# ruanjue/bsalign

Hardware: AMD Instinct MI355X
Metric: GCUPS (giga band-cell updates / s), 8-bit banded striped global alignment (higher is better)
Workload: dtype i8

## Files before the change

### bsalign_amd/__init__.py

```python
import ctypes as C
import os
import sys

import numpy as np

_HERE = os.path.dirname(os.path.abspath(__file__))
LIB_PATH = os.environ.get("BSA_LIB_PATH") or os.path.join(_HERE, "libbsalign_hip.so")

MODE_GLOBAL, MODE_OVERLAP, MODE_EXTEND = 0, 1, 2
MODE_ROWRECORDS, MODE_SCORE_ONLY, MODE_SEQ2BIT = 0x100, 0x400, 0x800
MODE_CIGAR_EQX = 0x1000
MODE_QSTRAND = 0x2000
MODE_BAND_MARGIN = 0x4000
ST_MARGIN_SHIFT, ST_MARGIN_NONE = 16, 0xFFFF
QOFF_REVCOMP = 1 << 63
CIGAR_M, CIGAR_I, CIGAR_D, CIGAR_EQ, CIGAR_X = 0, 1, 2, 7, 8
ST_BAD_BASE, ST_EMPTY, ST_TRACE, ST_DEVICE = 1, 2, 4, 8
KMER_CHAIN_DEVICE = 1
KMER_STRAND_AUTO = 2
ST_REVCOMP = 16
WINDOW_NONE = 0xFFFFFFFF

E_NAMES = {0: "OK", -1: "BSA_E_NODEVICE", -2: "BSA_E_ARG", -3: "BSA_E_NOMEM", -4: "BSA_E_HIP",
           -5: "BSA_E_CIGAR_CAP", -6: "BSA_E_UNSUPPORTED"}
# ... 51 lines not shown
class KmerParams(C.Structure):
    _fields_ = [("ksz", C.c_uint32), ("threads", C.c_uint32)]


RESULT_DTYPE = np.dtype([(n, np.int32) for n in ("score", "qb", "qe", "tb", "te", "mat", "mis", "ins", "del", "aln")])

_lib = None


DIAGDP_PROB_DTYPE = np.dtype([("seq0", np.uint64), ("seq1", np.uint64), ("mats0", np.uint64, (4,)), ("mats1", np.uint64, (4,)),
                              ("out0", np.uint64), ("out1", np.uint64), ("mlen", np.uint32), ("mbeg", np.uint32), ("mend", np.uint32), ("W", np.uint32)])


def build():
    import subprocess
    subprocess.run(["make", "-s", "-C", os.path.join(_HERE, "csrc"), "all"], check=True)


def lib():
    global _lib
    if _lib is None:
        if not os.path.exists(LIB_PATH):
            raise RuntimeError("libbsalign_hip.so is not built (run `python -c 'import __graft_entry__ as g; g.build()'`); "
                               "there is no CPU fallback")
        if "torch" not in sys.modules and not os.environ.get("BSA_NO_TORCH_PRELOAD"):
            try:
                import torch
            except ImportError:
                pass
        L = C.CDLL(LIB_PATH)
        vp, u8p, u32p, u64p = C.c_void_p, C.c_void_p, C.c_void_p, C.c_void_p
        L.bsa_ctx_create.argtypes = [C.c_int, C.POINTER(vp)]
        L.bsa_ctx_destroy.argtypes = [vp]
        L.bsa_ctx_destroy.restype = None
        L.bsa_ctx_set_stream.argtypes = [vp, vp]
        L.bsa_ctx_set_workspace_limit.argtypes = [vp, C.c_size_t]
        L.bsa_ctx_sync.argtypes = [vp]
        L.bsa_last_error.argtypes = [vp]
        L.bsa_last_error.restype = C.c_char_p
        L.bsa_ctx_last_kernel_ms.argtypes = [vp, C.POINTER(C.c_double), C.POINTER(C.c_long), C.POINTER(C.c_double)]
        L.bsa_ctx_last_trace_ms.argtypes = [vp, C.POINTER(C.c_double), C.POINTER(C.c_long)]
        L.bsa_ctx_last_margin_ms.argtypes = [vp, C.POINTER(C.c_double), C.POINTER(C.c_long)]
        L.bsa_ctx_last_kernel_name.argtypes = [vp, C.c_int]
        L.bsa_ctx_last_kernel_name.restype = C.c_char_p
        L.bsa_ctx_last_handover.argtypes = [vp]
        L.bsa_ctx_last_handover.restype = C.c_long
        L.bsa_set_score_matrix.argtypes = [C.POINTER(C.c_int8), C.c_int8, C.c_int8]
        L.bsa_set_score_matrix.restype = None
        L.bsa_align_batch.argtypes = [vp, u8p, C.c_size_t, u64p, u32p, u64p, u32p, C.c_size_t, C.POINTER(AlignParams),
                                      vp, u32p, C.c_size_t, u64p, u32p]
        L.bsa_align_plan_create.argtypes = [vp, u64p, u32p, u64p, u32p, C.c_size_t, C.POINTER(AlignParams), C.POINTER(vp)]
        if hasattr(L, "bsa_align8_abs_form_internal"):
            L.bsa_align8_abs_form_internal.argtypes = [C.POINTER(AlignParams), C.POINTER(C.c_uint32)]
        if hasattr(L, "bsa_align8_flag_span_internal"):
            L.bsa_align8_flag_span_internal.argtypes = [C.POINTER(AlignParams), C.POINTER(C.c_uint32)]
        if hasattr(L, "bsa_align8_x_choice_internal"):
            L.bsa_align8_x_choice_internal.argtypes = [C.POINTER(AlignParams), C.c_uint32, C.c_uint32, C.c_int, C.c_uint32, C.c_int, C.c_uint64, C.c_int,
                                                       C.POINTER(C.c_uint64), C.c_char_p, C.c_size_t]
        L.bsa_align_plan_destroy.argtypes = [vp]
        L.bsa_align_plan_destroy.restype = None
        L.bsa_align_plan_cells.argtypes = [vp]
        L.bsa_align_plan_cells.restype = C.c_double
        L.bsa_align_run.argtypes = [vp, u8p, vp, u32p, C.c_size_t, u64p, u32p]
        L.bsa_synth_stride.argtypes = [C.c_uint32]
        L.bsa_synth_stride.restype = C.c_size_t
        L.bsa_synth_pairs_host.argtypes = [C.c_uint64, C.c_uint64, C.c_size_t, C.c_uint32, C.c_uint32, u8p, u32p]
        L.bsa_synth_pairs_dev.argtypes = [vp, C.c_uint64, C.c_uint64, C.c_size_t, C.c_uint32, C.c_uint32, u8p, u32p]
        L.bsa_seq_pack2bit.argtypes = [vp, u8p, C.c_uint64, u64p, u32p]
        if hasattr(L, "bsa_edit_batch"):
            L.bsa_edit_batch.argtypes = [vp, u8p, C.c_size_t, u64p, u32p, u64p, u32p, C.c_size_t, C.POINTER(EditParams),
                                         vp, u32p, C.c_size_t, u64p, u32p]
            L.bsa_edit_plan_create.argtypes = [vp, u64p, u32p, u64p, u32p, C.c_size_t, C.POINTER(EditParams), C.POINTER(vp)]
            L.bsa_edit_plan_destroy.argtypes = [vp]
            L.bsa_edit_plan_destroy.restype = None
            L.bsa_edit_plan_cells.argtypes = [vp]
            L.bsa_edit_plan_cells.restype = C.c_double
            L.bsa_edit_run.argtypes = [vp, u8p, vp, u32p, C.c_size_t, u64p, u32p]
        if hasattr(L, "bsa_edit_choice_internal"):
            L.bsa_edit_choice_internal.argtypes = [C.c_uint32, C.c_uint32, C.c_uint32, C.c_int, C.c_uint32, C.c_int, C.c_int, C.c_int, C.c_int, C.c_int,
                                                   C.POINTER(C.c_uint64), C.c_char_p, C.c_char_p, C.c_size_t]
        L.bsa_kmer_edit_batch.argtypes = [vp, u8p, C.c_size_t, u64p, u32p, u64p, u32p, C.c_size_t, C.POINTER(KmerParams),
                                          vp, u32p, C.c_size_t, u64p, u32p]
        L.bsa_kmer_edit_batch2.argtypes = [vp, u8p, C.c_size_t, u64p, u32p, u64p, u32p, C.c_size_t, C.POINTER(KmerParams),
                                           vp, u32p, C.c_size_t, u64p, u32p, C.c_uint32]
        L.bsa_kmer_chain_batch.argtypes = [vp, u8p, C.c_size_t, u64p, u32p, u64p, u32p, C.c_size_t, C.c_uint32,
                                           u64p, C.c_size_t, u64p, u32p]
        L.bsa_kmer_chain_batch2.argtypes = [vp, u8p, C.c_size_t, u64p, u32p, u64p, u32p, C.c_size_t, C.c_uint32,
                                            u64p, C.c_size_t, u64p, u32p, C.c_uint32]
        L.bsa_ctx_last_kmer_chain_ms.argtypes = [vp, C.POINTER(C.c_double), C.POINTER(C.c_long), C.POINTER(C.c_long)]
        L.bsa_kmer_chain_plan_create.argtypes = [vp, u64p, u32p, u64p, u32p, C.c_size_t, C.c_uint32, C.c_uint32, C.POINTER(vp)]
        L.bsa_kmer_chain_plan_destroy.argtypes = [vp]
        L.bsa_kmer_chain_plan_destroy.restype = None
        L.bsa_kmer_chain_plan_chunks.argtypes = [vp]
        L.bsa_kmer_chain_plan_chunks.restype = C.c_uint32
        L.bsa_kmer_chain_words_bound.argtypes = [u32p, u32p, C.c_size_t]
        L.bsa_kmer_chain_words_bound.restype = C.c_uint64
        L.bsa_kmer_chain_run.argtypes = [vp, u8p, u64p, C.c_size_t, u64p, u32p]
        L.bsa_cigar_windows_bound.argtypes = [u32p, C.c_size_t, C.c_uint32]
        L.bsa_cigar_windows_bound.restype = C.c_uint64
        L.bsa_cigar_windows_run.argtypes = [vp, vp, u32p, u64p, C.c_size_t, C.c_uint32, vp, C.c_size_t, u64p]
        L.bsa_cigar_windows_batch.argtypes = [vp, vp, u32p, u64p, C.c_size_t, C.c_uint32, vp, C.c_size_t, u64p]
        L.bsa_rows_block_bytes.argtypes = [C.c_uint32, C.c_int8, C.c_int8, C.c_int8, C.c_int8]
        L.bsa_rows_block_bytes.restype = C.c_size_t
        L.bsa_rows_run.argtypes = [vp, vp, vp, C.c_size_t, vp, vp, vp, C.POINTER(RowsParams)]
        L.bsa_sweep_run.argtypes = [vp, vp, vp, vp, C.c_size_t, vp, vp, vp, C.POINTER(SweepParams), vp]
        L.bsa_sweep_host.argtypes = [vp, vp, C.c_size_t, vp, C.c_size_t, vp, vp, vp, C.c_size_t, C.POINTER(SweepParams), vp, C.c_size_t, vp]
        L.bsa_poa_graph_supported.argtypes = [C.POINTER(SweepParams), C.c_uint32]
        L.bsa_poa_graph_host.argtypes = [vp, vp, C.c_size_t, vp, C.c_size_t, vp, C.c_size_t, vp, C.c_size_t, vp, C.c_size_t, C.POINTER(SweepParams),
                                         vp, vp, C.c_size_t, vp, vp]
        L.bsa_poa_graph_run.argtypes = [vp, vp, C.c_size_t, vp, vp, vp, C.c_size_t, vp, C.c_uint32, C.POINTER(SweepParams), vp, vp, vp, vp, vp, vp]
        L.bsa_align_debug_rows.argtypes = [vp, C.c_uint32, u8p, C.c_size_t, C.POINTER(C.c_uint32)]
        L.bsa_diagdp_batch.argtypes = [vp, u8p, C.c_size_t, vp, C.c_size_t, u8p, C.c_size_t]
        L.bsa_diagdp_last_ms.argtypes = [vp]
        L.bsa_diagdp_last_ms.restype = C.c_double
        L.bsa_env_reload.restype = None
        _lib = L
    _sync_env()
    return _lib


_env_seen = None


def _sync_env():
    global _env_seen
    cur = tuple(sorted((k, v) for k, v in os.environ.items() if k.startswith("BSA_")))
    if cur != _env_seen:
        _lib.bsa_env_reload()
        _env_seen = cur


def _np(a, dt):
    return np.ascontiguousarray(a, dtype=dt)


def _p(a):
    return a.ctypes.data_as(C.c_void_p)


def make_params(mode=MODE_GLOBAL, bandwidth=128, M=2, X=-6, O=-3, E=-2, Q=0, P=0, matrix=None):
    p = AlignParams()
    p.mode, p.bandwidth = mode, bandwidth
    if matrix is None:
        lib().bsa_set_score_matrix(p.matrix, M, X)
    else:
        for i in range(16):
            p.matrix[i] = int(matrix[i])
    p.gapo1, p.gape1, p.gapo2, p.gape2 = O, E, Q, P
    return p


def align8_abs_form(par):
    rows = C.c_uint32(0)
    form = lib().bsa_align8_abs_form_internal(C.byref(par), C.byref(rows))
    return int(form), int(rows.value)


FLAG_SPAN_TERMS = ("M: f - d", "D: d - E", "D: f - E", "D: d - E, row -1", "D: f - E, row -1", "R, Od")


def align8_flag_span(par):
    terms = (C.c_uint32 * len(FLAG_SPAN_TERMS))()
    span = lib().bsa_align8_flag_span_internal(C.byref(par), terms)
    return int(span), tuple(int(v) for v in terms)


X_CHOICE_FIELDS = ("form", "W", "L", "pw", "do2", "score", "abs", "m3", "wps", "rebase_rows", "grid", "groups", "nseg", "seg_rows", "spin_cap", "rmask", "ctl_bytes",
                   "state_bytes", "n8", "nb8", "gap_model", "xq_need")
X_NONE, X_STATIC, X_SEG, X_WHOLE, X_MIX = range(5)


def align8_x_choice(par, count, max_tlen, static_band=False, code_fmt=0, score=False, xq_bytes=0, cus=256):
    out = (C.c_uint64 * len(X_CHOICE_FIELDS))()
    name = C.create_string_buffer(400)
    rc = lib().bsa_align8_x_choice_internal(C.byref(par), count, max_tlen, int(static_band), code_fmt, int(score), xq_bytes, cus, out, name, len(name))
    if rc < 0:
        raise ValueError("bsa_align8_x_choice_internal: bad arguments")
    d = dict(zip(X_CHOICE_FIELDS, (int(v) for v in out)))
    d.update(name=name.value.decode(), launch=rc == 1)
    return d


EDIT_CHOICE_FIELDS = tuple("fwd%d_%s" % (i, f) for i in (0, 1) for f in ("form", "n", "tiled", "track", "lanes", "grid", "block")) \
    + ("trace_form", "trace_tiled", "trace_lanes", "trace_grid", "row_fmt")
E_NONE, E_REG, E_GRP, E_GRP32, E_WIDE, E_GEN = range(6)
T_NONE, T_WAVE, T_PLAIN, T_COOP = range(4)


def edit_choice(bw, wide, count, mode=MODE_GLOBAL, bandwidth=0, score=False, alone=True, cus=256, occ_plain=8, occ_coop=8):
    out = (C.c_uint64 * len(EDIT_CHOICE_FIELDS))()
    fwd, trace = C.create_string_buffer(200), C.create_string_buffer(200)
    rc = lib().bsa_edit_choice_internal(bw, wide, count, mode, bandwidth, int(score), int(alone), cus, occ_plain, occ_coop, out, fwd, trace, 200)
    if rc < 0:
        raise ValueError("bsa_edit_choice_internal: bad arguments")
    d = dict(zip(EDIT_CHOICE_FIELDS, (int(v) for v in out)))
    d.update(fwd_name=fwd.value.decode(), trace_name=trace.value.decode(), launch=rc == 1)
    return d


def pack2bit(codes):
    c = np.ascontiguousarray(codes, dtype=np.uint8).ravel()
    nw = (c.size + 31) // 32
    buf = np.zeros(nw * 32, dtype=np.uint64)
    buf[:c.size] = c & 3
    shift = np.uint64(62) - np.uint64(2) * np.arange(32, dtype=np.uint64)
    return np.bitwise_or.reduce(buf.reshape(nw, 32) << shift, axis=1).astype(np.uint64)


def unpack2bit(words, off, n):
    i = np.uint64(off) + np.arange(n, dtype=np.uint64)
# ... 465 lines not shown
```

### bsalign_amd/csrc/bsa_align8_x.hip

```cpp
#include "bsa_common.h"
#include "bsa_dpp.h"
#include <algorithm>
#include <cstdio>
typedef short xv2s __attribute__((ext_vector_type(2)));
typedef unsigned short xv2u __attribute__((ext_vector_type(2)));
static __device__ __forceinline__ uint32_t x_add(uint32_t a, uint32_t b){ return __builtin_bit_cast(uint32_t, (xv2u)(__builtin_bit_cast(xv2u, a) + __builtin_bit_cast(xv2u, b))); }
static __device__ __forceinline__ uint32_t x_sub(uint32_t a, uint32_t b){ return __builtin_bit_cast(uint32_t, (xv2u)(__builtin_bit_cast(xv2u, a) - __builtin_bit_cast(xv2u, b))); }
static __device__ __forceinline__ uint32_t x_max(uint32_t a, uint32_t b){ return __builtin_bit_cast(uint32_t, __builtin_elementwise_max(__builtin_bit_cast(xv2s, a), __builtin_bit_cast(xv2s, b))); }
typedef _Float16 xv2h __attribute__((ext_vector_type(2)));
static __device__ __forceinline__ uint32_t x_max3(uint32_t a, uint32_t b, uint32_t c){
	return __builtin_bit_cast(uint32_t, __builtin_elementwise_maximum(__builtin_elementwise_maximum(__builtin_bit_cast(xv2h, a), __builtin_bit_cast(xv2h, b)), __builtin_bit_cast(xv2h, c)));
}
static __device__ __forceinline__ uint32_t x_minu(uint32_t a, uint32_t b){ return __builtin_bit_cast(uint32_t, __builtin_elementwise_min(__builtin_bit_cast(xv2u, a), __builtin_bit_cast(xv2u, b))); }
static __device__ __forceinline__ uint32_t x_satsubu(uint32_t a, uint32_t b){ return __builtin_bit_cast(uint32_t, __builtin_elementwise_sub_sat(__builtin_bit_cast(xv2u, a), __builtin_bit_cast(xv2u, b))); }
static __device__ __forceinline__ uint32_t x_acc(uint32_t acc, uint32_t flag, uint32_t two){
	return __builtin_bit_cast(uint32_t, (xv2u)(__builtin_bit_cast(xv2u, acc) * __builtin_bit_cast(xv2u, two) + __builtin_bit_cast(xv2u, flag)));
}
static __device__ __forceinline__ uint32_t x_ins(uint32_t acc, uint32_t n, uint32_t bit){ return __builtin_amdgcn_bitop3_b32(n, acc, bit, 0x4E); }
static __device__ __forceinline__ uint32_t x_ins0(uint32_t n, uint32_t bit){ return __builtin_amdgcn_bitop3_b32(n, n, bit, 0x0A); }
static __device__ __forceinline__ uint32_t x_shl15(uint32_t a){ return __builtin_bit_cast(uint32_t, (xv2u)(__builtin_bit_cast(xv2u, a) << 15)); }
static __device__ __forceinline__ uint32_t x_ashr8(uint32_t a){ return __builtin_bit_cast(uint32_t, (xv2s)(__builtin_bit_cast(xv2s, a) >> 8)); }
static __device__ __forceinline__ uint32_t x_shl8(uint32_t a){ return __builtin_bit_cast(uint32_t, (xv2u)(__builtin_bit_cast(xv2u, a) << 8)); }
static __device__ __forceinline__ void x_sel(uint32_t &x, uint32_t y, uint64_t take){ asm("v_cndmask_b32 %0, %0, %1, %2" : "+v"(x) : "v"(y), "s"(take)); }
static __device__ __forceinline__ uint32_t x_q8(int v){ return (((uint32_t)v & 0xffu) << 8) * 0x00010001u; }
static __device__ __forceinline__ uint32_t x_i16(int v){ return ((uint32_t)v & 0xffffu) * 0x00010001u; }
static __device__ __forceinline__ int x_lo8(uint32_t x){ return __builtin_amdgcn_sbfe((int)x, 8, 8); }
static __device__ __forceinline__ int x_hi8(uint32_t x){ return (int)x >> 24; }
static __device__ __forceinline__ int x_lo16(uint32_t x){ return __builtin_amdgcn_sbfe((int)x, 0, 16); }
static __device__ __forceinline__ int x_hi16(uint32_t x){ return (int)x >> 16; }

#define XDPP(old, x, ctrl, bank) ((uint32_t)__builtin_amdgcn_update_dpp((int)(old), (int)(x), (ctrl), 0xf, (bank), false))
#define XDPPZ(x, ctrl, bank) ((uint32_t)__builtin_amdgcn_update_dpp(0, (int)(x), (ctrl), 0xf, (bank), true))
#define XQP(a, b, c, d) ((a) | ((b) << 2) | ((c) << 4) | ((d) << 6))
#define XROW_SHL(n) (0x100 + (n))
#define XROW_SHR(n) (0x110 + (n))
#define XHALF_MIRROR 0x141

template<int L> static __device__ __forceinline__ uint32_t x_bcast_first(uint32_t x){
	const uint32_t s = XDPPZ(x, XQP(0, 0, 0, 0), 0xf);
	if constexpr (L == 4) return s;
	else return XDPP(s, s, XROW_SHR(4), 0xA);
}
template<int L> static __device__ __forceinline__ uint32_t x_bcast_last(uint32_t x){
	const uint32_t s = XDPPZ(x, XQP(3, 3, 3, 3), 0xf);
	if constexpr (L == 4) return s;
	else return XDPP(s, s, XROW_SHL(4), 0x5);
}
template<int L> static __device__ __forceinline__ uint32_t x_shift_down(uint32_t x, uint32_t fill_lo, bool first){
	if constexpr (L == 4){
		const uint32_t r = XDPPZ(x, XQP(3, 0, 1, 2), 0xf);
		return __builtin_amdgcn_perm(r, fill_lo, first ? 0x05040100u : 0x07060504u);
	}
	const uint32_t s = XDPPZ(x, XROW_SHR(1), 0xf);
	const uint32_t w = XDPPZ(x, XROW_SHL(L - 1), 0xf);
	const uint32_t fix = (w << 16) | (fill_lo & 0xffffu);
	return first ? fix : s;
}
template<int L> static __device__ __forceinline__ uint32_t x_shift_up(uint32_t x, uint32_t fill, bool last){
	if constexpr (L == 4){
		const uint32_t r = XDPPZ(x, XQP(1, 2, 3, 0), 0xf);
		return __builtin_amdgcn_perm(fill, r, last ? 0x05040302u : 0x03020100u);
	}
	const uint32_t s = XDPPZ(x, XROW_SHL(1), 0xf);
	const uint32_t w = XDPPZ(x, XROW_SHR(L - 1), 0xf);
	const uint32_t fix = __builtin_amdgcn_alignbit(fill, w, 16);
	return last ? fix : s;
}
template<int L> static __device__ __forceinline__ uint32_t x_scan_max(uint32_t x){
	uint32_t y = XDPP(x, x, XQP(0, 0, 2, 2), 0xf); x = x_max(x, y);
	y = XDPP(x, x, XQP(0, 1, 1, 1), 0xf); x = x_max(x, y);
	if constexpr (L == 8){
		const uint32_t z = XDPP(x, x, XQP(3, 3, 3, 3), 0xf);
		y = XDPP(x, z, XROW_SHR(4), 0xA); x = x_max(x, y);
	}
	return x;
}
// ... 715 lines not shown
		auto sb = [&](int q) -> uint32_t { return (uint32_t)(((int)a.matrix[q * 4 + t] - 2 * GE) & 0xff); };
		xa_mtab[2 * t] = (uint32_t)((BSA_EPI8_MIN - 2 * GE) & 0xff) | (sb(0) << 8) | (sb(1) << 24);
		xa_mtab[2 * t + 1] = (sb(2) << 8) | (sb(3) << 24);
	}
	__builtin_amdgcn_wave_barrier();

	uint32_t Hp[W], E[W];
	int base = 0;
	uint32_t svH = 0, svE = 0;
	uint32_t rbeg = 0, mov = 0, i = row0;
	int cand_sc = BSA_SCORE_MIN, cand_te = 0;
	const uint32_t NGP = ((uint32_t)(-GE * jl * W) & 0xffffu) | ((uint32_t)(-GE * (jl + L) * W) << 16);
	if(row0 == 0u){
		const int first_u = (int)(int8_t)(gapo1 + gape1 + a.smin - a.smax);
		const bool ov = mode == BSA_MODE_OVERLAP;
		base = (ov ? 0 : gapo1 + 2 * gape1) - FB;
#pragma unroll
		for(int k = 0; k < W; k++){
			Hp[k] = ov ? x_add(NGP, x_i16(FB + GE - GE * k)) : x_i16(FB);
			E[k] = ov ? x_add(NGP, x_i16(FB - GE * k - NE0)) : x_i16(FB - NE0);
		}
		if(last){
			const uint32_t hl = (Hp[W - 1] >> 16) + (uint32_t)(cfirst - GE - NEWNE);
			E[W - 1] = (E[W - 1] & 0xffffu) | (hl << 16);
		}
		svH = ov ? x_i16(FB + 2 * GE) : x_i16(FB + GE - first_u);
		svE = ov ? x_i16(FB + GE - NE0) : x_i16(FB - NE0);
	}
	if(row0 != 0u){
		const uint32_t *sp = st + (lt & 63);
		int r = 0;
#pragma unroll
		for(int k = 0; k < W; k++) Hp[k] = sp[64 * r++];
#pragma unroll
		for(int k = 0; k < W; k++) E[k] = sp[64 * r++];
		base = (int)sp[64 * r++]; svH = sp[64 * r++]; svE = sp[64 * r++];
		rbeg = sp[64 * r++]; mov = sp[64 * r++]; cand_sc = (int)sp[64 * r++]; cand_te = (int)sp[64 * r++];
	}
	__shared__ uint32_t xa_stage[EXT ? 1 : NWV][EXT ? 1 : 4 * ND][64];
	uint32_t *const stg = EXT ? ext_stage + (size_t)(lt >> 6) * (4 * ND * 64) + (lt & 63) : &xa_stage[(!EXT && NWV > 1) ? (lt >> 6) : 0][0][lt & 63];
	constexpr int KD = 4 + 12, NSEL = 2 * KD;
	constexpr uint32_t QOFFMAX = (uint32_t)(NSEL - W);
	static_assert(NSEL % 4 == 0 && NSEL - W <= BSA_QPAD_TAIL, "a refill reads NSEL - W bytes behind the band's last block");
	__shared__ uint32_t xa_qwin[EXT ? 1 : NWV][EXT ? 1 : 2 * KD][64];
	uint32_t *const qwp = EXT ? ext_qwin + (size_t)(lt >> 6) * (2 * KD * 64) + (lt & 63) : &xa_qwin[(!EXT && NWV > 1) ? (lt >> 6) : 0][0][lt & 63];
	uint32_t wbase = 0x40000000u;
	int begq = 0;
	if(tlen != 0u && first && row0 == 0u) begs[0] = 0;
	uint64_t twin = 0;
	if(row0 < tlen){ __builtin_memcpy(&twin, tp + row0, 8); twin <<= 3; }
	const int rbz = 2 * max((int)(tlen / max(qlen, 1u)), 1);
	const bool rush32 = (unsigned long long)(uint32_t)rbz * tlen + qlen + (uint32_t)BW + (uint32_t)rbz < 0xFFFFFFFFull;
	uint32_t rzl = rush32 ? (uint32_t)rbz * (tlen - min(row0, tlen) - 1u) : 0u;
	int rby_tab = 0;
	const int rby_lane = (lt & (64 - L)) << 2;

	uint64_t actm = 0;
	while(i < row1 && (actm = __builtin_amdgcn_ballot_w64(i < tlen)) != 0ull){
		const bool act = i < tlen;
		if(mode == BSA_MODE_GLOBAL && (i & (uint32_t)(L - 1)) == 0u)
			rby_tab = (int)((1.0 * (double)(i + (uint32_t)jl) / (double)tlen) * (double)qlen);
		if((i & rmask) == 0u){
			const uint32_t bc = x_bcast_first<L>(Hp[0]);
			const uint32_t dl = x_sub(__builtin_amdgcn_perm(bc, bc, 0x01000100u), x_i16(FB));
#pragma unroll
			for(int k = 0; k < W; k++){ Hp[k] = x_sub(Hp[k], dl); E[k] = x_sub(E[k], dl); }
			svH = x_sub(svH, dl); svE = x_sub(svE, dl);
			base += x_lo16(bc) - FB;
		}
		mov = min(mov, __builtin_elementwise_sub_sat(qlen, rbeg + (uint32_t)BW));
		rbeg += mov;
		int rhj = 0;
		if(__builtin_expect((__builtin_amdgcn_ballot_w64(mov != 1u) & actm) != 0ull, 0)){
			if(__any(act && mov >= (uint32_t)BW)){
				const bool z = act && mov >= (uint32_t)BW;
				const uint32_t bc = x_bcast_last<L>(Hp[W - 1]);
				const int rhz = base + x_hi16(bc) + GE * ((int)(rbeg - mov) + BW - 1 + (int)i - 1);
				if(z){
					rhj = rhz;
					base = BSA_SCORE_MIN - GE * ((int)rbeg + (int)i - 2) - FB;
#pragma unroll
					for(int k = 0; k < W; k++){ Hp[k] = x_add(NGP, x_i16(FB - GE * k)); E[k] = x_add(NGP, x_i16(FB - GE * (k + 1) - NEWNE)); }
				}
			}
			if(__any(act && mov == 0u)){
				const bool d = act && mov == 0u;
				const uint64_t dm = __ballot(d);
				const uint32_t pu = x_shift_down<L>(Hp[W - 1], svH, first), pe = x_shift_down<L>(E[W - 1], svE, first);
#pragma unroll
				for(int k = W - 1; k >= 1; k--){ x_sel(Hp[k], Hp[k - 1], dm); x_sel(E[k], E[k - 1], dm); }
				x_sel(Hp[0], pu, dm); x_sel(E[0], pe, dm);
			}
			for(uint32_t s = 1; __any(act && mov < (uint32_t)BW && s < mov); s++){
				const bool d = act && mov < (uint32_t)BW && s < mov;
				const uint64_t dm = __ballot(d);
				uint32_t hfill = __builtin_amdgcn_perm(Hp[W - 1], Hp[W - 1], 0x03020302u);
				if(s == 1u) hfill = x_add(hfill, ENT16);
				const uint32_t efill = __builtin_amdgcn_perm(E[W - 1], E[W - 1], 0x03020302u);
				const uint32_t inh = x_shift_up<L>(Hp[0], hfill, last), ine = x_shift_up<L>(E[0], efill, last);
#pragma unroll
				for(int k = 0; k + 1 < W; k++){ x_sel(Hp[k], Hp[k + 1], dm); x_sel(E[k], E[k + 1], dm); }
				x_sel(Hp[W - 1], inh, dm); x_sel(E[W - 1], ine, dm);
			}
		}
		uint32_t S[W];
		{
			const uint32_t tw32 = (i & 4u) ? (uint32_t)(twin >> 32) : (uint32_t)twin;
			const uint32_t tb8 = __builtin_amdgcn_ubfe(tw32, 8u * (i & 3u), 5u);
			uint32_t off = rbeg - wbase;
			if(__builtin_expect((__builtin_amdgcn_ballot_w64(off > QOFFMAX) & actm) != 0ull, 0)){
				if(act){
					const uint8_t *pl = qp + rbeg + jl * W, *ph = qp + rbeg + (jl + L) * W;
					uint32_t bl[NSEL / 4], bh[NSEL / 4];
					__builtin_memcpy(bl, pl, NSEL); __builtin_memcpy(bh, ph, NSEL);
					uint32_t TV = 0x07050301u, TS = 0x0B0A0908u;
					asm volatile("" : "+v"(TV), "+v"(TS));
#pragma unroll
					for(int n = 0; n < NSEL / 4; n++){
						const uint32_t lv = __builtin_amdgcn_perm(0x00000000u, TV, bl[n]), ls = __builtin_amdgcn_perm(0x0000000Du, TS, bl[n]);
						const uint32_t hv = __builtin_amdgcn_perm(0x00000000u, TV, bh[n]), hs = __builtin_amdgcn_perm(0x0000000Du, TS, bh[n]);
						const uint32_t l01 = __builtin_amdgcn_perm(ls, lv, 0x05010400u), l23 = __builtin_amdgcn_perm(ls, lv, 0x07030602u);
						const uint32_t h01 = __builtin_amdgcn_perm(hs, hv, 0x05010400u), h23 = __builtin_amdgcn_perm(hs, hv, 0x07030602u);
						qwp[64 * (4 * n)] = __builtin_amdgcn_perm(h01, l01, 0x05040100u);
						qwp[64 * (4 * n + 1)] = __builtin_amdgcn_perm(h01, l01, 0x07060302u);
						qwp[64 * (4 * n + 2)] = __builtin_amdgcn_perm(h23, l23, 0x05040100u);
						qwp[64 * (4 * n + 3)] = __builtin_amdgcn_perm(h23, l23, 0x07060302u);
					}
					wbase = rbeg; off = 0u;
				}
			}
			const uint32_t *wl = qwp + 64u * (act ? off : 0u);
			const uint2 mr = *(const uint2*)((const uint8_t*)xa_mtab + tb8);
#pragma unroll
			for(int k = 0; k < W; k++) S[k] = __builtin_amdgcn_perm(mr.y, mr.x, wl[64 * k]);
		}
		const uint32_t d0s = x_add(Hp[0], S[0]);
		uint32_t d0h = d0s;
		uint32_t q0m, q0d;
		asm volatile("" : "=v"(q0m), "=v"(q0d));
		const uint32_t fini = x_add(Hp[0], MINF16);
		if(__builtin_expect((__builtin_amdgcn_ballot_w64(mov - 1u >= (uint32_t)BW - 1u) & actm) != 0ull, 0)){
			const int hp0 = x_lo16(Hp[0]);
			const int HBr = base + hp0 + GE * ((int)rbeg + (int)i - 2);
			const bool near = mov == 0u && rbeg != 0u && HBr > BSA_SCORE_MIN + (1 << 17);
			if((__builtin_amdgcn_ballot_w64(mov - 1u >= (uint32_t)BW - 1u && !near) & actm) == 0ull){
				if(first && mov == 0u) d0h = (d0s & 0xffff0000u) | (fini & 0xffffu);
			} else {
				int rh;
				if(mov >= (uint32_t)BW) rh = rhj;
				else if(rbeg) rh = BSA_SCORE_MIN;
				else if(mode == BSA_MODE_OVERLAP || i == 0) rh = 0;
				else rh = gapo1 + gape1 * (int)i;
				const int s0 = x_lo16(S[0]) + 2 * GE;
				const int t0 = x_lo16(E[0]) - hp0 + 2 * GE;
				int hh = (rh - HBr) + s0;
// ... 144 lines not shown
				}
			} else {
				const uint32_t xm = __builtin_amdgcn_perm(accM[0], accM[1], 0x07030501u), xd = __builtin_amdgcn_perm(accD[0], accD[1], 0x07030501u);
				const uint32_t xr = __builtin_amdgcn_perm(accR[0], accR[1], 0x07030501u), xo = __builtin_amdgcn_perm(accO[0], accO[1], 0x07030501u);
				cur[0] = __builtin_amdgcn_perm(xd, xm, 0x05040100u); cur[1] = __builtin_amdgcn_perm(xo, xr, 0x05040100u);
				cur[2] = __builtin_amdgcn_perm(xd, xm, 0x07060302u); cur[3] = __builtin_amdgcn_perm(xo, xr, 0x07060302u);
			}
			const uint32_t ri = i & 3u;
			if constexpr (CWD == 1){
				uint32_t *const sr = stg + 64u * ri;
#pragma unroll
				for(int q = 0; q < ND; q++) sr[256 * q] = cur[q];
			} else {
				uint32_t *const sr = stg + (64u * ND) * ri;
#pragma unroll
				for(int q = 0; q < ND; q++) sr[64 * q] = cur[q];
			}
			if(act && (ri == 3u || i + 1u == tlen)){
				uint32_t *gp = (uint32_t*)rowp + bsa_code_off(i & ~3u, 0u, CWD);
				if constexpr (CWD == 1){
#pragma unroll
					for(int q = 0; q < ND; q++){
						const uint32_t blk = (uint32_t)(NACC * (jl + L * (q / NACC)) + q % NACC);
						uint4 t; t.x = stg[256 * q]; t.y = stg[256 * q + 64]; t.z = stg[256 * q + 128]; t.w = stg[256 * q + 192];
						*(uint4*)(gp + 4u * blk) = t;
					}
				} else {
#pragma unroll
					for(int hb = 0; hb < 2; hb++){
						uint32_t *bp = gp + (4u * CWD) * (uint32_t)(jl + L * hb);
#pragma unroll
						for(int pc = 0; pc < CWD; pc++){
							uint4 t;
							uint32_t *tw = (uint32_t*)&t;
#pragma unroll
							for(int e = 0; e < 4; e++){
								const int lin = 4 * pc + e, row = lin / CWD, d = lin % CWD;
								tw[e] = stg[64 * (ND * row + CWD * hb + d)];
							}
							*(uint4*)(bp + 4 * pc) = t;
						}
					}
				}
			}
		}
		const uint32_t hv = x_add(Hp[0], GE16);
		const uint32_t Hsh = x_shift_down<L>(Hp[W - 1], hv, first);
		const uint32_t bcl = x_bcast_last<L>(Hp[W - 1]);
		if(act){
			constexpr uint32_t LM = (uint32_t)(L - 1);
			const bool lastrow = i + 1u == tlen;
			if((i & LM) == (uint32_t)jl) begq = (int)rbeg;
			if(((i & LM) == LM || lastrow) && (uint32_t)jl <= (i & LM)) begs[(i & ~LM) + 1u + (uint32_t)jl] = begq;
			const int rbase = base + GE * ((int)rbeg + (int)i);
			auto score_at = [&](uint32_t pos) -> int {
				const uint32_t b = pos / W, kk = pos % W;
				const bool hi = b >= (uint32_t)L;
				uint32_t hh = Hp[0];
#pragma unroll
				for(int k = 1; k < W; k++) x_sel(hh, Hp[k], __ballot((uint32_t)k == kk));
				return rbase + (hi ? x_hi16(hh) : x_lo16(hh)) + GE * (int)pos;
			};
			if(mode != BSA_MODE_GLOBAL && rbeg + BW >= qlen){
				const uint32_t pos = qlen - 1u - rbeg;
				if(((pos / W) & (uint32_t)(L - 1)) == (uint32_t)jl){
					const int sc = score_at(pos);
					if(sc > cand_sc){ cand_sc = sc; cand_te = (int)i; }
				}
			}
			if(lastrow && mode == BSA_MODE_GLOBAL){
				const uint32_t pos = qlen - 1u - rbeg;
				int *const gs = begs + tlen + 1u;
				if(pos >= (uint32_t)BW){ if(first) *gs = (int)0x80000000u; }
				else if(((pos / W) & (uint32_t)(L - 1)) == (uint32_t)jl) *gs = score_at(pos);
			} else if(lastrow){
				bsa_code_end_t *er = (bsa_code_end_t*)(rowp + (size_t)bsa_code_rows(tlen) * (64u * CWD));
#pragma unroll
				for(int q = 0; q < 16 / L; q++){ er->cand_sc[jl + L * q] = q ? BSA_SCORE_MIN : cand_sc; er->cand_te[jl + L * q] = q ? 0 : cand_te; }
				int8_t *ub = (int8_t*)(er + 1);
#pragma unroll
				for(int hf = 0; hf < 2; hf++){
					const int b = jl + L * hf;
					auto half = [&](uint32_t x) -> int { return hf ? x_hi16(x) : x_lo16(x); };
					er->ubegs[b * CR] = rbase + half(Hsh) + GE * (b * W - 1);
					if constexpr (CR == 2) er->ubegs[b * CR + 1] = rbase + half(Hp[W / 2 - 1]) + GE * (b * W + W / 2 - 1);
#pragma unroll
					for(int k = 0; k < W; k++) ub[b * W + k] = (int8_t)(half(Hp[k]) - half((k == 0) ? Hsh : Hp[k - 1]) + GE);
				}
				if(last){ er->ubegs[16] = rbase + x_hi16(Hp[W - 1]) + GE * (BW - 1); er->rbeg_last = (int)rbeg; }
			}
		}
		{
			uint32_t x;
			if constexpr (CR == 1){
				const uint32_t dl = x_add(x_sub(Hp[W - 1], Hsh), x_i16(W * GE));
				x = x_max(dl, x_sub(0u, dl));
			} else {
				const uint32_t HGE16 = x_i16((W / 2) * GE);
				const uint32_t da = x_add(x_sub(Hp[W / 2 - 1], Hsh), HGE16), db = x_add(x_sub(Hp[W - 1], Hp[W / 2 - 1]), HGE16);
				x = x_add(x_max(da, x_sub(0u, da)), x_max(db, x_sub(0u, db)));
			}
			x = x_sum<L>(x);
			const int nzsum = (int)((x & 0xffffu) + (x >> 16));
			const uint32_t bcf = x_bcast_first<L>(Hp[0]);
			const int d16 = x_hi16(bcl) - x_lo16(bcf) + (BW - 1) * GE;
			uint32_t nz = (uint32_t)(nzsum / 16);
			nz = nz / (uint32_t)WR * 16u / 2u;
			const int noisy = (int)((16u > nz) ? 16u : nz);
			int rbx;
			if(i <= (uint32_t)BW / 4u) rbx = 0;
			else if(rbeg + BW >= qlen) rbx = 0;
			else if(noisy < d16) rbx = 2;
			else if(d16 < -noisy) rbx = 0;
			else rbx = 1;
			if(mode == BSA_MODE_GLOBAL){
				const int rby = __builtin_amdgcn_ds_bpermute(rby_lane + (int)((i & (uint32_t)(L - 1)) << 2), rby_tab);
				const uint32_t left = tlen - i - 1u;
				bool rush;
				if(rush32) rush = act && rbeg + rzl + (uint32_t)BW <= qlen + (uint32_t)rbz - 1u;
				else {
					const unsigned long long lhs = (unsigned long long)rbeg + (unsigned long long)(uint32_t)rbz * left + (unsigned long long)BW;
					rush = act && lhs <= (unsigned long long)(uint32_t)(qlen + (uint32_t)rbz - 1u);
				}
				if((int)rbeg < rby - BW) mov = (uint32_t)(rbx + 1);
				else if((int)rbeg > rby) mov = (uint32_t)max(0, rbx - 1);
				else mov = (uint32_t)rbx;
				if(rush) mov = 1u + (uint32_t)(qlen - (rbeg + BW)) / max(left, 1u);
			} else mov = (uint32_t)rbx;
		}
		{
			const uint32_t efill = x_add(__builtin_amdgcn_perm(Hp[W - 1], Hp[W - 1], 0x03020302u), x_i16(cfirst - GE - NEWNE));
			E[W - 1] = x_shift_up<L>(tmpE0, efill, last);
			svH = hv; svE = tmpE0;
		}
		i++;
		rzl -= (uint32_t)rbz;
		if((i & 7u) == 0u && i < tlen){ __builtin_memcpy(&twin, tp + i, 8); twin <<= 3; }
	}
	if(st != nullptr && row1 < tlen){
		uint32_t *sp = st + (lt & 63);
		int r = 0;
		auto put = [&](uint32_t v){ __hip_atomic_store(sp + 64 * r, v, __ATOMIC_RELAXED, __HIP_MEMORY_SCOPE_AGENT); r++; };
#pragma unroll
		for(int k = 0; k < W; k++) put(Hp[k]);
#pragma unroll
		for(int k = 0; k < W; k++) put(E[k]);
		put((uint32_t)base); put(svH); put(svE);
		put(rbeg); put(mov); put((uint32_t)cand_sc); put((uint32_t)cand_te);
	}
}
template<int L, int PW, bool DO2, bool M3 = true>
__global__ void __launch_bounds__(256) __attribute__((amdgpu_waves_per_eu(3))) k_align8_fwd_x_abs(const Align8Args a, const uint32_t rmask){
	x_forward_abs<L, 4, PW, DO2, false, M3>(a, a.first, a.count, blockIdx.x * 256u, rmask);
}

template<int W, int L, bool DO2 = false, bool SCORE = false>
__global__ void __launch_bounds__(256) k_align8_fwd_x(const Align8Args a){
	x_forward<W, L, 1, false, 4, DO2, false, SCORE>(a, a.first, a.count, blockIdx.x * 256u);
}
template<int W, int L, bool SCORE = false>
__global__ void __launch_bounds__(256) k_align8_fwd_x0(const Align8Args a){
	x_forward<W, L, 0, false, 4, false, false, SCORE>(a, a.first, a.count, blockIdx.x * 256u);
}
__global__ void __launch_bounds__(256) k_align8_fwd_x2(const Align8Args a){
	x_forward<8, 8, 2>(a, a.first, a.count, blockIdx.x * 256u);
}
template<int W, int L>
__global__ void __launch_bounds__(256) k_align8_fwd_x2w(const Align8Args a){
	x_forward<W, L, 2>(a, a.first, a.count, blockIdx.x * 256u);
// ... 236 lines not shown

constexpr uint32_t x_key(uint32_t form, uint32_t W, uint32_t L, int pw, bool do2, bool score, bool abs, bool m3, uint32_t wps){
	return form | W << 3 | L << 8 | (uint32_t)pw << 12 | (uint32_t)do2 << 14 | (uint32_t)score << 15 | (uint32_t)abs << 16 | (uint32_t)m3 << 17 | wps << 18;
}
#define X_STATIC_K(W, L, PW, DO2, SCORE) case x_key(X_STATIC, W, L, PW, DO2, SCORE, false, false, 3): hipLaunchKernelGGL((k_align8_fwd_x_static<W, L, PW, DO2, SCORE>), grid, dim3(256), 0, st, a); break;
#define X_SEG_K(W, L, PW, DO2, WPS, SCORE, ABS, M3) case x_key(X_SEG, W, L, PW, DO2, SCORE, ABS, M3, WPS): hipLaunchKernelGGL((k_align8_fwd_xq<W, L, PW, DO2, WPS, SCORE, ABS, M3>), grid, dim3(64), 0, st, a, q); break;
#define X_ABS_K(L, PW, DO2, M3) case x_key(X_WHOLE, 16, L, PW, DO2, false, true, M3, 3): hipLaunchKernelGGL((k_align8_fwd_x_abs<L, PW, DO2, M3>), grid, dim3(256), 0, st, a, rmask); break;
#define X_K1(W, L, DO2, SCORE) case x_key(X_WHOLE, W, L, 1, DO2, SCORE, false, false, 3): hipLaunchKernelGGL((k_align8_fwd_x<W, L, DO2, SCORE>), grid, dim3(256), 0, st, a); break;
#define X_K0(W, L, SCORE) case x_key(X_WHOLE, W, L, 0, false, SCORE, false, false, 3): hipLaunchKernelGGL((k_align8_fwd_x0<W, L, SCORE>), grid, dim3(256), 0, st, a); break;
#define X_K2W(W, L) case x_key(X_WHOLE, W, L, 2, false, false, false, false, 3): hipLaunchKernelGGL((k_align8_fwd_x2w<W, L>), grid, dim3(256), 0, st, a); break;
#define X_MIX_K(ABS) case x_key(X_MIX, 16, 4, 1, false, false, ABS, ABS, 3): hipLaunchKernelGGL(k_align8_fwd_x_mix<ABS>, grid, dim3(256), 0, st, a, l.nb8, l.n8, ABS ? rmask : 0u); break;
static hipError_t x_run(const XLaunch &l, const Align8Args &a, hipStream_t st){
	XQArgs q = l.q;
	if(l.form == X_SEG){
		q.ctl = a.xq; q.state = (uint32_t*)((uint8_t*)a.xq + l.ctl_bytes);
		const hipError_t err = hipMemsetAsync(a.xq, 0, l.ctl_bytes, st);
		if(err != hipSuccess) return err;
	}
	const dim3 grid(l.grid);
	const uint32_t rmask = l.rebase_rows - 1u;
	switch(x_key(l.form, l.W, l.L, l.pw, l.do2, l.score, l.abs, l.m3, l.wps)){
		X_STATIC_K(8, 4, 0, false, false) X_STATIC_K(16, 4, 0, false, false) X_STATIC_K(16, 8, 0, false, false)
		X_STATIC_K(8, 4, 0, false, true) X_STATIC_K(16, 4, 0, false, true) X_STATIC_K(16, 8, 0, false, true)
		X_STATIC_K(8, 4, 1, false, false) X_STATIC_K(16, 4, 1, false, false) X_STATIC_K(16, 8, 1, false, false)
		X_STATIC_K(8, 4, 1, false, true) X_STATIC_K(16, 4, 1, false, true) X_STATIC_K(16, 8, 1, false, true)
		X_STATIC_K(16, 4, 1, true, false) X_STATIC_K(8, 8, 2, false, false)
		X_SEG_K(8, 4, 0, false, 3, false, false, false) X_SEG_K(16, 4, 0, false, 3, false, false, false) X_SEG_K(16, 8, 0, false, 3, false, false, false)
		X_SEG_K(8, 4, 1, false, 3, false, false, false) X_SEG_K(16, 4, 1, false, 3, false, false, false) X_SEG_K(16, 8, 1, false, 3, false, false, false)
		X_SEG_K(8, 4, 0, false, 3, true, false, false) X_SEG_K(16, 4, 0, false, 3, true, false, false) X_SEG_K(16, 8, 0, false, 3, true, false, false)
		X_SEG_K(8, 4, 1, false, 3, true, false, false) X_SEG_K(16, 4, 1, false, 3, true, false, false) X_SEG_K(16, 8, 1, false, 3, true, false, false)
		X_SEG_K(16, 4, 0, false, 3, false, true, true) X_SEG_K(16, 8, 0, false, 3, false, true, true) X_SEG_K(16, 8, 0, false, 3, false, true, false)
		X_SEG_K(16, 4, 1, false, 3, false, true, true) X_SEG_K(16, 8, 1, false, 3, false, true, true) X_SEG_K(16, 8, 1, false, 3, false, true, false)
		X_SEG_K(16, 4, 1, true, 3, false, false, false) X_SEG_K(16, 4, 1, true, 3, false, true, true)
		X_SEG_K(8, 4, 2, false, 3, false, false, false) X_SEG_K(8, 8, 2, false, 3, false, false, false) X_SEG_K(16, 4, 2, false, 2, false, false, false)
		X_ABS_K(4, 0, false, true) X_ABS_K(8, 0, false, true) X_ABS_K(8, 0, false, false)
		X_ABS_K(4, 1, false, true) X_ABS_K(8, 1, false, true) X_ABS_K(8, 1, false, false) X_ABS_K(4, 1, true, true)
		X_K1(4, 8, false, false) X_K1(8, 4, false, false) X_K1(8, 8, false, false) X_K1(16, 4, false, false) X_K1(16, 8, false, false)
		X_K1(16, 4, true, false) X_K1(8, 4, false, true) X_K1(16, 4, false, true) X_K1(16, 8, false, true)
		X_K0(4, 8, false) X_K0(8, 4, false) X_K0(16, 4, false) X_K0(16, 8, false) X_K0(8, 4, true) X_K0(16, 4, true) X_K0(16, 8, true)
		X_K2W(8, 4) X_K2W(16, 8) case x_key(X_WHOLE, 8, 8, 2, false, false, false, false, 3): hipLaunchKernelGGL(k_align8_fwd_x2, grid, dim3(256), 0, st, a); break;
		X_MIX_K(false) X_MIX_K(true)
		default: return hipErrorInvalidValue;
	}
	if(l.name) bsa_last_fwd_kernel = l.name;
	return hipGetLastError();
}
static hipError_t x_launch(const Align8Args &a, int pw, bool score, hipStream_t st){
	if(a.count == 0) return hipSuccess;
	const XLaunch l = x_choose(a, pw, score, bsa_cus());
	return l.form == X_NONE ? hipErrorInvalidValue : x_run(l, a, st);
}
hipError_t bsa_launch_align8_fwd_x(const Align8Args &a, int pw, hipStream_t st){ return x_launch(a, pw, false, st); }
hipError_t bsa_launch_align8_fwd_x_score(const Align8Args &a, int pw, hipStream_t st){ return x_launch(a, pw, true, st); }
```

Measured before the change: 2534.

## Replace per-row double division with incremental row target; use per-lane slot shifts

The per-row band target (a*qlen/tlen in double precision) is now advanced incrementally with an integer quotient/remainder step. It falls back to the exact double expression when the remainder hits zero or the sizes are wide, so results stay bit-identical. The band-move slot shifts switch from ballot-masked per-register cndmask chains to predicated packed v_pk_mov shifts. The last-row/overlap score bookkeeping is wrapped in a wave-uniform unlikely branch, and a host-side test hook for the row-target arithmetic is added.

```diff
diff --git a/bsalign_amd/__init__.py b/bsalign_amd/__init__.py
--- a/bsalign_amd/__init__.py
+++ b/bsalign_amd/__init__.py
@@ -127,6 +127,9 @@
         L.bsa_align_plan_create.argtypes = [vp, u64p, u32p, u64p, u32p, C.c_size_t, C.POINTER(AlignParams), C.POINTER(vp)]
         if hasattr(L, "bsa_align8_abs_form_internal"):
             L.bsa_align8_abs_form_internal.argtypes = [C.POINTER(AlignParams), C.POINTER(C.c_uint32)]
+        if hasattr(L, "bsa_align8_row_target_internal"):
+            L.bsa_align8_row_target_internal.argtypes = [C.POINTER(C.c_uint32), C.POINTER(C.c_uint32), C.POINTER(C.c_uint32), C.c_size_t, C.c_uint32, C.c_uint32,
+                                                         C.POINTER(C.c_int32), C.POINTER(C.c_uint8)]
         if hasattr(L, "bsa_align8_flag_span_internal"):
             L.bsa_align8_flag_span_internal.argtypes = [C.POINTER(AlignParams), C.POINTER(C.c_uint32)]
         if hasattr(L, "bsa_align8_x_choice_internal"):
@@ -231,6 +234,19 @@
     return int(form), int(rows.value)
 
 
+def align8_row_target(a, tlen, qlen, stride=4, steps=0):
+    import numpy as np
+    a, tlen, qlen = (np.ascontiguousarray(x, dtype=np.uint32) for x in (a, tlen, qlen))
+    assert a.shape == tlen.shape == qlen.shape and a.ndim == 1
+    value, fb = np.empty(len(a), np.int32), np.empty(len(a), np.uint8)
+    u32p = C.POINTER(C.c_uint32)
+    rc = lib().bsa_align8_row_target_internal(a.ctypes.data_as(u32p), tlen.ctypes.data_as(u32p), qlen.ctypes.data_as(u32p), len(a), stride, steps,
+                                              value.ctypes.data_as(C.POINTER(C.c_int32)), fb.ctypes.data_as(C.POINTER(C.c_uint8)))
+    if rc != 0:
+        raise ValueError("align8_row_target: a row outside its target or a target of length 0")
+    return value, fb.astype(bool)
+
+
 FLAG_SPAN_TERMS = ("M: f - d", "D: d - E", "D: f - E", "D: d - E, row -1", "D: f - E, row -1", "R, Od")
 
 
diff --git a/bsalign_amd/csrc/bsa_align8_x.hip b/bsalign_amd/csrc/bsa_align8_x.hip
--- a/bsalign_amd/csrc/bsa_align8_x.hip
+++ b/bsalign_amd/csrc/bsa_align8_x.hip
@@ -22,6 +22,58 @@
 static __device__ __forceinline__ uint32_t x_ashr8(uint32_t a){ return __builtin_bit_cast(uint32_t, (xv2s)(__builtin_bit_cast(xv2s, a) >> 8)); }
 static __device__ __forceinline__ uint32_t x_shl8(uint32_t a){ return __builtin_bit_cast(uint32_t, (xv2u)(__builtin_bit_cast(xv2u, a) << 8)); }
 static __device__ __forceinline__ void x_sel(uint32_t &x, uint32_t y, uint64_t take){ asm("v_cndmask_b32 %0, %0, %1, %2" : "+v"(x) : "v"(y), "s"(take)); }
+typedef uint32_t xv2w __attribute__((ext_vector_type(2)));
+template<int W> static __device__ __forceinline__ void x_slots_up(uint32_t *X, uint32_t in){
+	xv2w P[W / 2];
+#pragma unroll
+	for(int j = 0; j < W / 2; j++){ P[j].x = X[2 * j]; P[j].y = X[2 * j + 1]; }
+#pragma unroll
+	for(int j = W / 2 - 1; j >= 1; j--) asm("v_pk_mov_b32 %0, %1, %0 op_sel:[1,0]" : "+v"(P[j]) : "v"(P[j - 1]));
+	xv2w I;
+	I.x = in;
+	asm("v_pk_mov_b32 %0, %1, %0 op_sel:[0,0]" : "+v"(P[0]) : "v"(I));
+#pragma unroll
+	for(int j = 0; j < W / 2; j++){ X[2 * j] = P[j].x; X[2 * j + 1] = P[j].y; }
+}
+template<int W> static __device__ __forceinline__ void x_slots_down(uint32_t *X, uint32_t in){
+	xv2w P[W / 2];
+#pragma unroll
+	for(int j = 0; j < W / 2; j++){ P[j].x = X[2 * j]; P[j].y = X[2 * j + 1]; }
+#pragma unroll
+	for(int j = 0; j + 1 < W / 2; j++) asm("v_pk_mov_b32 %0, %0, %1 op_sel:[1,0]" : "+v"(P[j]) : "v"(P[j + 1]));
+	xv2w I;
+	I.x = in;
+	asm("v_pk_mov_b32 %0, %0, %1 op_sel:[1,0]" : "+v"(P[W / 2 - 1]) : "v"(I));
+#pragma unroll
+	for(int j = 0; j < W / 2; j++){ X[2 * j] = P[j].x; X[2 * j + 1] = P[j].y; }
+}
+static __host__ __device__ inline int x_rt_double(uint32_t a, uint32_t t, uint32_t q){ return (int)((1.0 * (double)a / (double)t) * (double)q); }
+struct XRowTgt { uint32_t k, r; };
+static __host__ __device__ inline bool x_rt_wide(uint32_t t, uint32_t q){ return (uint64_t)t * q >= (1ull << 52) || ((t | q) >> 31) != 0u; }
+static __host__ __device__ inline XRowTgt x_rt_at(uint32_t a, uint32_t t, uint32_t q){
+	XRowTgt s = {0u, 0u};
+	if(t == 0u) return s;
+	const uint64_t p = (uint64_t)a * q;
+	const double y = (double)p / (double)t;
+	uint32_t k = y < 4294967295.0 ? (uint32_t)y : 0u;
+	int64_t r = (int64_t)(p - (uint64_t)k * t);
+	if(r < 0){ k--; r += t; }
+	s.k = k; s.r = (uint32_t)r;
+	return s;
+}
+static __host__ __device__ inline void x_rt_step(XRowTgt &s, const XRowTgt &d, uint32_t t){
+	s.k += d.k; s.r += d.r;
+	if(s.r >= t){ s.r -= t; s.k++; }
+}
+static __host__ __device__ inline void x_rt_back(XRowTgt &s, const XRowTgt &d, uint32_t t){
+	s.k -= d.k;
+	if(s.r < d.r){ s.r += t; s.k--; }
+	s.r -= d.r;
+}
+static __host__ __device__ inline void x_rt_set(XRowTgt &s, uint32_t y, uint32_t t){
+	s.r += (s.k - y) * t;
+	s.k = y;
+}
 static __device__ __forceinline__ uint32_t x_q8(int v){ return (((uint32_t)v & 0xffu) << 8) * 0x00010001u; }
 static __device__ __forceinline__ uint32_t x_i16(int v){ return ((uint32_t)v & 0xffffu) * 0x00010001u; }
 static __device__ __forceinline__ int x_lo8(uint32_t x){ return __builtin_amdgcn_sbfe((int)x, 8, 8); }
@@ -843,14 +895,25 @@
 	const int rbz = 2 * max((int)(tlen / max(qlen, 1u)), 1);
 	const bool rush32 = (unsigned long long)(uint32_t)rbz * tlen + qlen + (uint32_t)BW + (uint32_t)rbz < 0xFFFFFFFFull;
 	uint32_t rzl = rush32 ? (uint32_t)rbz * (tlen - min(row0, tlen) - 1u) : 0u;
-	int rby_tab = 0;
+	XRowTgt rt = {0u, 0u}, rtd = {0u, 0u};
+	if(mode == BSA_MODE_GLOBAL){
+		rt = x_rt_at(row0 + (uint32_t)jl, tlen, qlen);
+		rtd = x_rt_at((uint32_t)L, tlen, qlen);
+		x_rt_back(rt, rtd, tlen);
+	}
+	const uint64_t rtwide = __builtin_amdgcn_ballot_w64(x_rt_wide(tlen, qlen));
 	const int rby_lane = (lt & (64 - L)) << 2;
 
 	uint64_t actm = 0;
 	while(i < row1 && (actm = __builtin_amdgcn_ballot_w64(i < tlen)) != 0ull){
 		const bool act = i < tlen;
-		if(mode == BSA_MODE_GLOBAL && (i & (uint32_t)(L - 1)) == 0u)
-			rby_tab = (int)((1.0 * (double)(i + (uint32_t)jl) / (double)tlen) * (double)qlen);
+		if(mode == BSA_MODE_GLOBAL && (i & (uint32_t)(L - 1)) == 0u){
+			x_rt_step(rt, rtd, tlen);
+			if(__builtin_expect(((__builtin_amdgcn_ballot_w64(rt.r == 0u) & __builtin_amdgcn_ballot_w64(i + (uint32_t)jl < tlen)) | (rtwide & actm)) != 0ull, 0)){
+				const uint32_t y = (uint32_t)x_rt_double(i + (uint32_t)jl, tlen, qlen);
+				x_rt_set(rt, y, tlen);
+			}
+		}
 		if((i & rmask) == 0u){
 			const uint32_t bc = x_bcast_first<L>(Hp[0]);
 			const uint32_t dl = x_sub(__builtin_amdgcn_perm(bc, bc, 0x01000100u), x_i16(FB));
@@ -876,22 +939,16 @@
 			}
 			if(__any(act && mov == 0u)){
 				const bool d = act && mov == 0u;
-				const uint64_t dm = __ballot(d);
 				const uint32_t pu = x_shift_down<L>(Hp[W - 1], svH, first), pe = x_shift_down<L>(E[W - 1], svE, first);
-#pragma unroll
-				for(int k = W - 1; k >= 1; k--){ x_sel(Hp[k], Hp[k - 1], dm); x_sel(E[k], E[k - 1], dm); }
-				x_sel(Hp[0], pu, dm); x_sel(E[0], pe, dm);
+				if(d){ x_slots_up<W>(Hp, pu); x_slots_up<W>(E, pe); }
 			}
 			for(uint32_t s = 1; __any(act && mov < (uint32_t)BW && s < mov); s++){
 				const bool d = act && mov < (uint32_t)BW && s < mov;
-				const uint64_t dm = __ballot(d);
 				uint32_t hfill = __builtin_amdgcn_perm(Hp[W - 1], Hp[W - 1], 0x03020302u);
 				if(s == 1u) hfill = x_add(hfill, ENT16);
 				const uint32_t efill = __builtin_amdgcn_perm(E[W - 1], E[W - 1], 0x03020302u);
 				const uint32_t inh = x_shift_up<L>(Hp[0], hfill, last), ine = x_shift_up<L>(E[0], efill, last);
-#pragma unroll
-				for(int k = 0; k + 1 < W; k++){ x_sel(Hp[k], Hp[k + 1], dm); x_sel(E[k], E[k + 1], dm); }
-				x_sel(Hp[W - 1], inh, dm); x_sel(E[W - 1], ine, dm);
+				if(d){ x_slots_down<W>(Hp, inh); x_slots_down<W>(E, ine); }
 			}
 		}
 		uint32_t S[W];
@@ -1142,42 +1199,44 @@
 			const bool lastrow = i + 1u == tlen;
 			if((i & LM) == (uint32_t)jl) begq = (int)rbeg;
 			if(((i & LM) == LM || lastrow) && (uint32_t)jl <= (i & LM)) begs[(i & ~LM) + 1u + (uint32_t)jl] = begq;
-			const int rbase = base + GE * ((int)rbeg + (int)i);
-			auto score_at = [&](uint32_t pos) -> int {
-				const uint32_t b = pos / W, kk = pos % W;
-				const bool hi = b >= (uint32_t)L;
-				uint32_t hh = Hp[0];
-#pragma unroll
-				for(int k = 1; k < W; k++) x_sel(hh, Hp[k], __ballot((uint32_t)k == kk));
-				return rbase + (hi ? x_hi16(hh) : x_lo16(hh)) + GE * (int)pos;
-			};
-			if(mode != BSA_MODE_GLOBAL && rbeg + BW >= qlen){
-				const uint32_t pos = qlen - 1u - rbeg;
-				if(((pos / W) & (uint32_t)(L - 1)) == (uint32_t)jl){
-					const int sc = score_at(pos);
-					if(sc > cand_sc){ cand_sc = sc; cand_te = (int)i; }
-				}
-			}
-			if(lastrow && mode == BSA_MODE_GLOBAL){
-				const uint32_t pos = qlen - 1u - rbeg;
-				int *const gs = begs + tlen + 1u;
-				if(pos >= (uint32_t)BW){ if(first) *gs = (int)0x80000000u; }
-				else if(((pos / W) & (uint32_t)(L - 1)) == (uint32_t)jl) *gs = score_at(pos);
-			} else if(lastrow){
-				bsa_code_end_t *er = (bsa_code_end_t*)(rowp + (size_t)bsa_code_rows(tlen) * (64u * CWD));
-#pragma unroll
-				for(int q = 0; q < 16 / L; q++){ er->cand_sc[jl + L * q] = q ? BSA_SCORE_MIN : cand_sc; er->cand_te[jl + L * q] = q ? 0 : cand_te; }
-				int8_t *ub = (int8_t*)(er + 1);
-#pragma unroll
-				for(int hf = 0; hf < 2; hf++){
-					const int b = jl + L * hf;
-					auto half = [&](uint32_t x) -> int { return hf ? x_hi16(x) : x_lo16(x); };
-					er->ubegs[b * CR] = rbase + half(Hsh) + GE * (b * W - 1);
-					if constexpr (CR == 2) er->ubegs[b * CR + 1] = rbase + half(Hp[W / 2 - 1]) + GE * (b * W + W / 2 - 1);
-#pragma unroll
-					for(int k = 0; k < W; k++) ub[b * W + k] = (int8_t)(half(Hp[k]) - half((k == 0) ? Hsh : Hp[k - 1]) + GE);
-				}
-				if(last){ er->ubegs[16] = rbase + x_hi16(Hp[W - 1]) + GE * (BW - 1); er->rbeg_last = (int)rbeg; }
+			if(__builtin_expect(__builtin_amdgcn_ballot_w64(lastrow || (mode != BSA_MODE_GLOBAL && rbeg + BW >= qlen)) != 0ull, 0)){
+				const int rbase = base + GE * ((int)rbeg + (int)i);
+				auto score_at = [&](uint32_t pos) -> int {
+					const uint32_t b = pos / W, kk = pos % W;
+					const bool hi = b >= (uint32_t)L;
+					uint32_t hh = Hp[0];
+#pragma unroll
+					for(int k = 1; k < W; k++) x_sel(hh, Hp[k], __ballot((uint32_t)k == kk));
+					return rbase + (hi ? x_hi16(hh) : x_lo16(hh)) + GE * (int)pos;
+				};
+				if(mode != BSA_MODE_GLOBAL && rbeg + BW >= qlen){
+					const uint32_t pos = qlen - 1u - rbeg;
+					if(((pos / W) & (uint32_t)(L - 1)) == (uint32_t)jl){
+						const int sc = score_at(pos);
+						if(sc > cand_sc){ cand_sc = sc; cand_te = (int)i; }
+					}
+				}
+				if(lastrow && mode == BSA_MODE_GLOBAL){
+					const uint32_t pos = qlen - 1u - rbeg;
+					int *const gs = begs + tlen + 1u;
+					if(pos >= (uint32_t)BW){ if(first) *gs = (int)0x80000000u; }
+					else if(((pos / W) & (uint32_t)(L - 1)) == (uint32_t)jl) *gs = score_at(pos);
+				} else if(lastrow){
+					bsa_code_end_t *er = (bsa_code_end_t*)(rowp + (size_t)bsa_code_rows(tlen) * (64u * CWD));
+#pragma unroll
+					for(int q = 0; q < 16 / L; q++){ er->cand_sc[jl + L * q] = q ? BSA_SCORE_MIN : cand_sc; er->cand_te[jl + L * q] = q ? 0 : cand_te; }
+					int8_t *ub = (int8_t*)(er + 1);
+#pragma unroll
+					for(int hf = 0; hf < 2; hf++){
+						const int b = jl + L * hf;
+						auto half = [&](uint32_t x) -> int { return hf ? x_hi16(x) : x_lo16(x); };
+						er->ubegs[b * CR] = rbase + half(Hsh) + GE * (b * W - 1);
+						if constexpr (CR == 2) er->ubegs[b * CR + 1] = rbase + half(Hp[W / 2 - 1]) + GE * (b * W + W / 2 - 1);
+#pragma unroll
+						for(int k = 0; k < W; k++) ub[b * W + k] = (int8_t)(half(Hp[k]) - half((k == 0) ? Hsh : Hp[k - 1]) + GE);
+					}
+					if(last){ er->ubegs[16] = rbase + x_hi16(Hp[W - 1]) + GE * (BW - 1); er->rbeg_last = (int)rbeg; }
+				}
 			}
 		}
 		{
@@ -1204,7 +1263,7 @@
 			else if(d16 < -noisy) rbx = 0;
 			else rbx = 1;
 			if(mode == BSA_MODE_GLOBAL){
-				const int rby = __builtin_amdgcn_ds_bpermute(rby_lane + (int)((i & (uint32_t)(L - 1)) << 2), rby_tab);
+				const int rby = __builtin_amdgcn_ds_bpermute(rby_lane + (int)((i & (uint32_t)(L - 1)) << 2), (int)rt.k);
 				const uint32_t left = tlen - i - 1u;
 				bool rush;
 				if(rush32) rush = act && rbeg + rzl + (uint32_t)BW <= qlen + (uint32_t)rbz - 1u;
@@ -1547,3 +1606,25 @@
 }
 hipError_t bsa_launch_align8_fwd_x(const Align8Args &a, int pw, hipStream_t st){ return x_launch(a, pw, false, st); }
 hipError_t bsa_launch_align8_fwd_x_score(const Align8Args &a, int pw, hipStream_t st){ return x_launch(a, pw, true, st); }
+
+extern "C" int bsa_align8_row_target_internal(const uint32_t *a, const uint32_t *tlen, const uint32_t *qlen, size_t n, uint32_t stride, uint32_t steps, int32_t *value, uint8_t *fallback){
+	if(!a || !tlen || !qlen || !value || !fallback || (steps != 0u && stride == 0u)) return -1;
+	for(size_t j = 0; j < n; j++){
+		const uint32_t t = tlen[j], q = qlen[j];
+		if(t == 0u || a[j] >= t) return -1;
+		if(x_rt_wide(t, q)){ fallback[j] = 1; value[j] = x_rt_double(a[j], t, q); continue; }
+		const uint32_t back = steps ? std::min(steps, a[j] / stride) : 0u;
+		XRowTgt s = x_rt_at(a[j] - back * stride, t, q);
+		if(back){
+			const XRowTgt d = x_rt_at(stride, t, q);
+			x_rt_back(s, d, t);
+			for(uint32_t m = 0; m <= back; m++){
+				x_rt_step(s, d, t);
+				if(s.r == 0u && m < back) x_rt_set(s, (uint32_t)x_rt_double(a[j] - (back - m) * stride, t, q), t);
+			}
+		}
+		fallback[j] = s.r == 0u;
+		value[j] = s.r == 0u ? x_rt_double(a[j], t, q) : (int32_t)s.k;
+	}
+	return 0;
+}
```

New measurement: 2612, median of 6. 1.03x the previous value.
